# DarylFernandes99/custom-yolo-implmentation

Hardware: AMD Instinct MI355X
Metric: images/sec (640x640 bf16) (higher is better)
Workload: dtype bf16; 1 GPU; preset s (width 32..512, depth 1) 640x640 train step (fwd+DFL/QFL loss+bwd+grad sync+AdamW), COCO-80 synthetic, 32 img/GPU; global_batch=32, parallelism=dp1, hip_graph=True, optimizer_in_graph=True, deterministic_mode=False

## Files before the change

custom-yolo-implmentation_amd/csrc/elementwise.hip:

```cpp
#include "common.h"

namespace {

constexpr int TPB = 256;
constexpr int RS_ROWS = 2;
constexpr int RS_MAXBLK = 256 * 8;

template <typename T> __host__ bool vec_ok(const void* p, long ld, int C) {
    constexpr int V = vec_of<T>::N;
    return (C % V == 0) && (ld % V == 0) && ((reinterpret_cast<uintptr_t>(p) % 16) == 0);
}

template <typename TI, typename TO>
__global__ void k_ncm_to_nhwc(const TI* __restrict__ src, long sn, long sc, long off,
                              TO* __restrict__ dst, int ld, int C, int HW) {
    __shared__ float tile[32][33];
    const int n = blockIdx.z, p0 = blockIdx.x * 32, c0 = blockIdx.y * 32;
    const int tx = threadIdx.x & 31, ty = threadIdx.x >> 5;
    for (int r = ty; r < 32; r += 8) {
        int c = c0 + r, p = p0 + tx;
        tile[r][tx] = (c < C && p < HW) ? to_f<TI>(src[n * sn + c * sc + off + p]) : 0.f;
    }
    __syncthreads();
    for (int r = ty; r < 32; r += 8) {
        int p = p0 + r, c = c0 + tx;
        if (p < HW && c < C) dst[((long)n * HW + p) * ld + c] = from_f<TO>(tile[tx][r]);
    }
}

template <typename TI, typename TO>
__global__ void k_nhwc_to_ncm(const TI* __restrict__ src, int ld, TO* __restrict__ dst, long sn,
                              long sc, long off, int C, int HW) {
    __shared__ float tile[32][33];
// ... 121 lines not shown
        int cg = (int)(i - p * cv);
        float a[V];
        load_pack<T, V>(src + p * lds_ + cg * V, a);
        if (ACC) {
            float b[V];
            load_pack<T, V>(dst + p * ldd + cg * V, b);
#pragma unroll
            for (int j = 0; j < V; ++j) a[j] += b[j];
        }
        store_pack<T, V>(dst + p * ldd + cg * V, a);
    }
}

struct AddSrcs { const void* p[4]; int ld[4]; };
template <typename T, int V, int NS>
__global__ void k_add_n(AddSrcs s, T* __restrict__ dst, int ldd, long npix, int cv) {
    long total = npix * cv;
    for (long i = blockIdx.x * (long)blockDim.x + threadIdx.x; i < total; i += (long)gridDim.x * blockDim.x) {
        long p = i / cv;
        int cg = (int)(i - p * cv);
        float a[V];
        load_pack<T, V>((const T*)s.p[0] + p * s.ld[0] + cg * V, a);
#pragma unroll
        for (int k = 1; k < NS; ++k) {
            float b[V];
            load_pack<T, V>((const T*)s.p[k] + p * s.ld[k] + cg * V, b);
#pragma unroll
            for (int j = 0; j < V; ++j) a[j] += b[j];
        }
        store_pack<T, V>(dst + p * ldd + cg * V, a);
    }
}

__device__ __forceinline__ float sigmoid_rcp(float x) { return __builtin_amdgcn_rcpf(1.0f + __expf(-x)); }

__device__ __forceinline__ float act_grad(float z, int act) {
    if (act == 0) return 1.f;
    float s = sigmoid_rcp(z);
    return s * (1.f + z * (1.f - s));
}
__device__ __forceinline__ float act_fwd(float z, int act) { return act == 0 ? z : z * sigmoid_rcp(z); }

struct RsThread { int rpb, r, cl, cg; bool active; };
__device__ __forceinline__ RsThread rs_thread(int tpr, int cv) {
    RsThread t;
    t.rpb = TPB / tpr;
    t.r = threadIdx.x / tpr;
    t.cl = threadIdx.x - t.r * tpr;
    t.cg = blockIdx.y * tpr + t.cl;
    t.active = (t.r < t.rpb) && (t.cg < cv);
    return t;
}

template <typename T, int V, typename F>
__device__ __forceinline__ void rs_walk(const RsThread& t, const T* __restrict__ a, int lda, const T* __restrict__ b, int ldb, bool has_b,
                                        long npix, F one) {
    const long step = (long)gridDim.x * t.rpb;
    long p = (long)blockIdx.x * t.rpb + t.r;
    for (; p + (RS_ROWS - 1) * step < npix; p += RS_ROWS * step) {
        pack_t<T, V> ra[RS_ROWS], rb[RS_ROWS];
#pragma unroll
        for (int k = 0; k < RS_ROWS; ++k) {
            ra[k] = load_raw<T, V>(a + (p + k * step) * lda + t.cg * V);
            if (has_b) rb[k] = load_raw<T, V>(b + (p + k * step) * ldb + t.cg * V);
        }
#pragma unroll
        for (int k = 0; k < RS_ROWS; ++k) one(p + k * step, ra[k], rb[k]);
    }
#pragma clang loop vectorize(disable)
    for (; p < npix; p += step) {
        pack_t<T, V> pa = load_raw<T, V>(a + p * lda + t.cg * V), pb;
        if (has_b) pb = load_raw<T, V>(b + p * ldb + t.cg * V);
        one(p, pa, pb);
// ... 21 lines not shown
            unpack<T, V>(pa, a);
            if (MODE == 1) unpack<T, V>(pd, d);
#pragma unroll
            for (int j = 0; j < V; ++j) {
                if (MODE == 0) { s[j] += a[j]; q[j] += a[j] * a[j]; }
                else {
                    float dz = d[j] * act_grad(a[j] * sc[j] + sh[j], ACT);
                    s[j] += dz;
                    q[j] += dz * a[j];
                }
            }
        });
    }
#pragma unroll
    for (int j = 0; j < V; ++j) { red[threadIdx.x][j] = s[j]; red[threadIdx.x][V + j] = q[j]; }
    __syncthreads();
    for (int t = threadIdx.x; t < tpr * 2 * V; t += TPB) {
        const int cl = t / (2 * V), j = t - cl * 2 * V;
        float a = 0.f;
#pragma unroll 8
        for (int rr = 0; rr < th.rpb; ++rr) a += red[rr * tpr + cl][j];
        const int cgo = blockIdx.y * tpr + cl;
        if (cgo < cv) sink((j / V) * C + cgo * V + (j % V), a);
    }
}

template <typename T, int V, int MODE, int ACT>
__global__ __launch_bounds__(TPB) __attribute__((amdgpu_waves_per_eu(5, 8)))
void k_channel_reduce(const T* __restrict__ y, int ldy, const T* __restrict__ dout, int ldd, const float* __restrict__ scale,
                      const float* __restrict__ shift, long npix, int C, float* __restrict__ partial, int tpr) {
    float* o = partial + (long)blockIdx.x * 2 * C;
    channel_sums<T, V, MODE, ACT>(y, ldy, dout, ldd, scale, shift, npix, C, tpr, [&](int i, float a) { o[i] = a; });
}

struct PIn {
    const void* p; int dt;
    __device__ __forceinline__ float ld(int i) const {
        return dt == YOLO_F32 ? ((const float*)p)[i] : dt == YOLO_BF16 ? (float)((const bf16_t*)p)[i] : (float)((const f16_t*)p)[i];
    }
};
struct PIo {
    void* p; int dt;
    __device__ __forceinline__ float ld(int i) const {
        return dt == YOLO_F32 ? ((const float*)p)[i] : dt == YOLO_BF16 ? (float)((const bf16_t*)p)[i] : (float)((const f16_t*)p)[i];
    }
    __device__ __forceinline__ void st(int i, float v) const {
        if (dt == YOLO_F32) ((float*)p)[i] = v; else if (dt == YOLO_BF16) ((bf16_t*)p)[i] = (bf16_t)v; else ((f16_t*)p)[i] = (f16_t)v;
    }
};
static inline bool pdt_ok(int dt) { return dt == YOLO_F32 || dt == YOLO_BF16 || dt == YOLO_F16; }

constexpr int BN_REPL = 8;

extern __shared__ float cf[];

__device__ __forceinline__ void acc_fold(const float* __restrict__ acc, int C, int c, double& s, double& q) {
    s = 0.0; q = 0.0;
#pragma unroll
    for (int r = 0; r < BN_REPL; ++r) { s += acc[(long)r * 2 * C + c]; q += acc[(long)r * 2 * C + C + c]; }
}

template <typename T, int V, int MODE, int ACT>
__global__ __launch_bounds__(TPB) __attribute__((amdgpu_waves_per_eu(5, 8)))
void k_channel_acc(const T* __restrict__ y, int ldy, const T* __restrict__ dout, int ldd, const float* __restrict__ scale,
                   const float* __restrict__ shift, long npix, int C, float* __restrict__ acc, int tpr) {
    float* o = acc + (long)(blockIdx.x % BN_REPL) * 2 * C;
    channel_sums<T, V, MODE, ACT>(y, ldy, dout, ldd, scale, shift, npix, C, tpr, [&](int i, float a) { atomicAdd(o + i, a); });
}

struct BnFwdCoef { float mean, invstd, scale, shift, unbiased; };
__device__ __forceinline__ BnFwdCoef bn_fwd_coef(double s, double q, float count, float eps, float gamma, float beta) {
    const double m = s / count;
    double var = q / count - m * m;
    if (var < 0.0) var = 0.0;
    BnFwdCoef k;
    k.invstd = (float)(1.0 / sqrt(var + (double)eps));
    k.mean = (float)m;
    k.scale = gamma * k.invstd;
    k.shift = beta - (float)m * k.scale;
    k.unbiased = (float)(count > 1.f ? var * (count / (count - 1.0)) : var);
    return k;
}
__device__ __forceinline__ void bn_fwd_publish(const BnFwdCoef& k, int c, float momentum, float* __restrict__ mean,
                                               float* __restrict__ invstd, float* __restrict__ scale,
                                               float* __restrict__ shift, const PIo& rmean, const PIo& rvar) {
    mean[c] = k.mean;
    invstd[c] = k.invstd;
    scale[c] = k.scale;
    shift[c] = k.shift;
    if (rmean.p) {
        rmean.st(c, (1.f - momentum) * rmean.ld(c) + momentum * k.mean);
        rvar.st(c, (1.f - momentum) * rvar.ld(c) + momentum * k.unbiased);
    }
}
struct BnBwdCoef { float dbeta, dgamma, A, B, D; };
__device__ __forceinline__ BnBwdCoef bn_bwd_coef(double s, double q, float count, const PIn& gamma, const float* __restrict__ mean,
                                                 const float* __restrict__ invstd, int c) {
    const double is = invstd[c], mu = mean[c];
    q = is * (q - mu * s);
    const double k0 = (double)gamma.ld(c) * is, c1 = s / count, c2 = q / count;
    BnBwdCoef k;
    k.dbeta = (float)s;
    k.dgamma = (float)q;
    k.A = (float)k0;
    k.B = (float)(-k0 * c2 * is);
    k.D = (float)(-k0 * c1 + k0 * c2 * mu * is);
    return k;
}

__global__ void k_bn_finalize_acc(const float* __restrict__ acc, float count, int C, const void* __restrict__ gamma_,
                                  const void* __restrict__ beta_, void* __restrict__ rmean_, void* __restrict__ rvar_,
                                  float momentum, float eps, float* __restrict__ mean, float* __restrict__ invstd,
                                  float* __restrict__ scale, float* __restrict__ shift, int pdt, int bdt) {
    const PIn gamma{gamma_, pdt}; const PIn beta{beta_, pdt}; const PIo rmean{rmean_, bdt}, rvar{rvar_, bdt};
    const int c = blockIdx.x * blockDim.x + threadIdx.x;
    if (c >= C) return;
    double s, q;
    acc_fold(acc, C, c, s, q);
    bn_fwd_publish(bn_fwd_coef(s, q, count, eps, gamma.ld(c), beta.ld(c)), c, momentum, mean, invstd, scale, shift, rmean, rvar);
}

template <typename T, int V>
__device__ __forceinline__ void bn_act_fwd_rows(const RsThread& th, const T* __restrict__ y, int ldy, const T* __restrict__ res,
                                                int ldr, T* __restrict__ out, int ldo, long npix, const float (&sc)[V],
                                                const float (&sh)[V], int act) {
    const bool has_res = res;
    rs_walk<T, V>(th, y, ldy, res, ldr, has_res, npix, [&](long p, const pack_t<T, V>& pa, const pack_t<T, V>& pt) {
        float a[V], t[V];
        unpack<T, V>(pa, a);
        if (has_res) unpack<T, V>(pt, t);
#pragma unroll
        for (int j = 0; j < V; ++j) a[j] = act_fwd(a[j] * sc[j] + sh[j], act) + (has_res ? t[j] : 0.f);
        store_pack<T, V>(out + p * ldo + th.cg * V, a);
    });
}

template <typename T, int V>
__device__ __forceinline__ void bn_act_bwd_rows(const RsThread& th, const T* __restrict__ dout, int ldd, const T* __restrict__ y,
                                                int ldy, T* __restrict__ dy, int lddy, long npix, int cw, int act) {
    const float* my = cf + th.cl * V;
// ... 699 lines not shown
```

custom-yolo-implmentation_amd/csrc/stem.hip:

```cpp
#include "common.h"
#include "conv_dev.h"

namespace {

template <typename TI, typename TO>
__global__ void k_stem_im2col(const TI* __restrict__ img, TO* __restrict__ col, int N, int H, int W, int OH, int OW) {
    long total = (long)N * OH * OW;
    for (long p = blockIdx.x * (long)blockDim.x + threadIdx.x; p < total; p += (long)gridDim.x * blockDim.x) {
        int ow = (int)(p % OW);
        long t = p / OW;
        int oh = (int)(t % OH);
        long n = t / OH;
        float v[32];
#pragma unroll
        for (int k = 27; k < 32; ++k) v[k] = 0.f;
#pragma unroll
        for (int ci = 0; ci < 3; ++ci) {
            const TI* plane = img + (n * 3 + ci) * (long)H * W;
#pragma unroll
            for (int kh = 0; kh < 3; ++kh) {
                int ih = 2 * oh + kh - 1;
#pragma unroll
                for (int kw = 0; kw < 3; ++kw) {
                    int iw = 2 * ow + kw - 1;
                    bool ok = ih >= 0 && ih < H && iw >= 0 && iw < W;
                    v[ci * 9 + kh * 3 + kw] = ok ? to_f<TI>(plane[(long)ih * W + iw]) : 0.f;
                }
            }
        }
        TO* o = col + p * 32;
        constexpr int V = vec_of<TO>::N;
#pragma unroll
        for (int k = 0; k < 32; k += V) {
// ... 269 lines not shown
    const int e = blockIdx.x * 8 + (threadIdx.x >> 5), l = threadIdx.x & 31;
    if (e >= Cout * 27) return;
    const int o = e / 27, k = e - o * 27;
    float s = 0.f;
    for (int b = l; b < nslab; b += 32) s += part[((long)b * Cout + o) * 32 + k];
#pragma unroll
    for (int off = 16; off > 0; off >>= 1) s += __shfl_xor(s, off, 32);
    if (l == 0) dw[e] = from_f<P>(s);
}

constexpr int STEM_WG_SLABS = 1024;

template <typename T>
int launch_stem_wgrad(const float* img, const void* dy, int ldy, float* part, int N, int H, int W, int OH, int OW, int Cout,
                      int* nslab, hipStream_t st) {
    const long tiles = (long)N * ((OH + 1) / 2) * ((OW + STEM_SEG - 1) / STEM_SEG);
    if (tiles <= 0) return YOLO_ERR_ARG;
    const int grid = (int)(tiles < STEM_WG_SLABS ? tiles : STEM_WG_SLABS);
    *nslab = grid;
#define STEM_WG(CT) hipLaunchKernelGGL((k_stem_wgrad<T, CT>), dim3(grid), dim3(256), 0, st, img, (const T*)dy, ldy, part, N, H, W, OH, OW, tiles)
    switch (Cout / 16) {
        case 1: STEM_WG(1); break;
        case 2: STEM_WG(2); break;
        case 3: STEM_WG(3); break;
        case 4: STEM_WG(4); break;
        case 6: STEM_WG(6); break;
        case 8: STEM_WG(8); break;
        default: return YOLO_ERR_ARG;
    }
#undef STEM_WG
    return YOLO_LAUNCH_CHECK();
}

template <typename T>
int launch_stem_conv(const float* img, const void* wp, void* y, int ldy, float* stats, int N, int H, int W, int OH, int OW,
                     int Cout, const float* bias, int act, hipStream_t st) {
    const long blocks = (long)N * ((OH + 1) / 2) * ((OW + STEM_SEG - 1) / STEM_SEG);
    if (blocks <= 0 || blocks > 0x7fffffffL) return YOLO_ERR_ARG;
#define STEM_CT(CT) hipLaunchKernelGGL((k_stem_conv<T, CT>), dim3((unsigned)blocks), dim3(256), 0, st, img, (const T*)wp, (T*)y, ldy, stats, N, H, W, OH, OW, Cout, bias, act)
    switch (Cout / 16) {
        case 1: STEM_CT(1); break;
        case 2: STEM_CT(2); break;
        case 3: STEM_CT(3); break;
        case 4: STEM_CT(4); break;
        case 6: STEM_CT(6); break;
        case 8: STEM_CT(8); break;
        default: return YOLO_ERR_ARG;
    }
#undef STEM_CT
    return YOLO_LAUNCH_CHECK();
}

}

extern "C" {

int yolo_stem_im2col(const void* img, int img_dtype, void* col, int col_dtype, int N, int H, int W, int OH, int OW,
                     hipStream_t st) {
    if (OH != (H - 1) / 2 + 1 || OW != (W - 1) / 2 + 1) return YOLO_ERR_ARG;
    long total = (long)N * OH * OW;
    int grid = (int)((total + 255) / 256 > 256 * 16 ? 256 * 16 : (total + 255) / 256);
    if (grid < 1) grid = 1;
#define STEM_LAUNCH(TI) YOLO_DISPATCH_T(col_dtype, hipLaunchKernelGGL((k_stem_im2col<TI, T>), dim3(grid), dim3(256), 0, st, (const TI*)img, (T*)col, N, H, W, OH, OW))
    switch (img_dtype) {
        case YOLO_F32:  STEM_LAUNCH(float); break;
        case YOLO_BF16: STEM_LAUNCH(bf16_t); break;
// ... 34 lines not shown
           (ct == 1 || ct == 2 || ct == 3 || ct == 4 || ct == 6 || ct == 8);
}

int yolo_stem_conv_fwd(const float* img, const void* wp, void* y, int ldy, float* stats, int N, int H, int W, int OH, int OW,
                       int Cout, const float* bias, int act, int dtype, hipStream_t st) {
    if ((bias != nullptr || act) && stats != nullptr) return YOLO_ERR_ARG;
    if (act != 0 && act != 1) return YOLO_ERR_ARG;
    if (!yolo_stem_conv_eligible(YOLO_F32, dtype, Cout) || ldy < Cout) return YOLO_ERR_ARG;
    if (OH != (H - 1) / 2 + 1 || OW != (W - 1) / 2 + 1) return YOLO_ERR_ARG;
    if (dtype == YOLO_BF16) return launch_stem_conv<bf16_t>(img, wp, y, ldy, stats, N, H, W, OH, OW, Cout, bias, act, st);
    return launch_stem_conv<f16_t>(img, wp, y, ldy, stats, N, H, W, OH, OW, Cout, bias, act, st);
}

int yolo_stem_wgrad_slabs(void) { return STEM_WG_SLABS; }

int yolo_stem_wgrad(const float* img, const void* dy, int ldy, float* partial, void* dw, int dw_dtype, int N, int H, int W,
                    int OH, int OW, int Cout, int dtype, hipStream_t st) {
    if (!yolo_stem_conv_eligible(YOLO_F32, dtype, Cout) || ldy < Cout || (ldy & 7) || (reinterpret_cast<uintptr_t>(dy) & 15)) return YOLO_ERR_ARG;
    if (OH != (H - 1) / 2 + 1 || OW != (W - 1) / 2 + 1) return YOLO_ERR_ARG;
    int nslab = 0;
    const int rc = dtype == YOLO_BF16 ? launch_stem_wgrad<bf16_t>(img, dy, ldy, partial, N, H, W, OH, OW, Cout, &nslab, st)
                                      : launch_stem_wgrad<f16_t>(img, dy, ldy, partial, N, H, W, OH, OW, Cout, &nslab, st);
    if (rc) return rc;
    const int grid = (Cout * 27 + 7) / 8;
    switch (dw_dtype) {
        case YOLO_F32:  hipLaunchKernelGGL((k_stem_wgrad_reduce<float>), dim3(grid), dim3(256), 0, st, partial, nslab, Cout, (float*)dw); break;
        case YOLO_BF16: hipLaunchKernelGGL((k_stem_wgrad_reduce<bf16_t>), dim3(grid), dim3(256), 0, st, partial, nslab, Cout, (bf16_t*)dw); break;
        case YOLO_F16:  hipLaunchKernelGGL((k_stem_wgrad_reduce<f16_t>), dim3(grid), dim3(256), 0, st, partial, nslab, Cout, (f16_t*)dw); break;
        default: return YOLO_ERR_DTYPE;
    }
    return YOLO_LAUNCH_CHECK();
}

}
```

custom-yolo-implmentation_amd/src/hipops/functions.py:

```python
import contextlib
import os

import torch

from . import ops
from .lib import ACT_IDENTITY, ACT_SILU

_LOWP = (torch.bfloat16, torch.float16)


def compute_dtype(x, w):
    dev = x.device.type
    if torch.is_autocast_enabled(dev):
        return torch.get_autocast_dtype(dev)
    if w.dtype in _LOWP:
        return w.dtype
    return x.dtype if x.dtype in (torch.float32,) + _LOWP else torch.float32


def _as_nhwc(t, dtype):
    return t if (t.dtype == dtype and ops.is_nhwc(t)) else ops.to_nhwc(t, dtype)


def _f32(t):
# ... 251 lines not shown


def fanout(x, k):
    if k < 2 or not (torch.is_grad_enabled() and x.requires_grad):
        return (x,) * k
    return Fanout.apply(x, k)


def _on_fwd_stream(forward):
    def on_stream(ctx, *args):
        if FWD_STREAM is not None:
            with torch.cuda.stream(FWD_STREAM):
                return forward(ctx, *args)
        return forward(ctx, *args)
    return staticmethod(on_stream)


def _bn_act_grads(dout, y, saved, act, training, acc_b):
    scale, shift, mean, invstd, gamma = saved
    if training and acc_b is not None:
        return ops.bn_act_bwd_train(dout, y, scale, shift, mean, invstd, gamma, act, acc_b)
    if training:
        return ops.bn_act_bwd(dout, y, scale, shift, mean, invstd, gamma, act)
    return ops.bn_act_bwd_eval(dout, y, scale, shift, act), None, None


def _stem_grads(x, weight, dy, fused):
    def run(out=None):
        if fused:
            return ops.stem_wgrad(x, dy, weight.dtype, out)
        return ops.stem_unpack_wgrad(ops.conv_wgrad(x, dy, 1, 1, torch.float32), weight.dtype, out)
    lazy = x.is_cuda and LAZY_WGRAD_JOIN
    return _param_grad(x.device, weight.shape, weight.dtype, (x, dy), run) if lazy else run()


def _dw_grads(x, weight, dy, xshape, link, want_dx, want_dw):
    dx = dw = None
    if want_dx:
        dx = _fan_bwd(link, xshape, dy.dtype, lambda into: ops.dw_dgrad(dy, _f32(weight).reshape(-1, 9), acc_into=into))
    if want_dw:
        if weight.dtype == torch.float32 and x.is_cuda and LAZY_WGRAD_JOIN:
            dw = _param_grad(x.device, (x.shape[1], 1, 3, 3), torch.float32, (x, dy), lambda out: ops.dw_wgrad(x, dy, out=out))
        else:
            dw = ops.dw_wgrad(x, dy).to(weight.dtype)
    return dx, dw


def _dense_dgrad(weight, dy, xshape, k, stride, link):
    (n, cin, h, w), T = xshape, dy.dtype
    def run(acc_into, acc2=None):
        return ops.conv_dgrad(dy, ops.pack_weights(weight, k, stride, 1, T), cin, h, w, k, stride, acc_into=acc_into, acc2=acc2)
    if link is not None and link.chunk is not None and link.chunk.absorb(link, xshape, T, stride, run):
        return None
    return _fan_bwd(link, xshape, T, run, leaves=link is not None and link.fan)


def _dense_grads(x, weight, dy, xshape, k, stride, link, want_dx, want_dw):
    if want_dx and want_dw:
        return _wgrad_overlapped(x, dy, k, stride, weight.dtype, lambda: _dense_dgrad(weight, dy, xshape, k, stride, link))
    if want_dx:
        return _dense_dgrad(weight, dy, xshape, k, stride, link), None
    return None, (ops.conv_wgrad(x, dy, k, stride, weight.dtype) if want_dw else None)


class ConvBnAct(torch.autograd.Function):

# ... 22 lines not shown
            y = ops.dw_fwd(x, _f32(weight).reshape(cout, 9), acc_f)
        else:
            x = _as_nhwc(x, T)
            y = ops.conv_fwd(x, ops.pack_weights(weight, k, stride, 0, T), None, cout, k, stride, acc_f)
        rm, rv = bufs
        if res is not None:
            res = _as_nhwc(res, T)
        acc_b = None
        if training:
            if BnArena.current is not None and not deterministic:
                acc_b = BnArena.current.take(cout)
            if deterministic:
                mean, invstd, scale, shift = ops.bn_train_stats(y, gamma, beta, rm, rv, momentum, eps)
                out = ops.bn_act_fwd(y, scale, shift, act, res, out)
            else:
                out, mean, invstd, scale, shift = ops.bn_act_fwd_train(y, acc_f, gamma, beta, rm, rv, momentum, eps, act, res, out)
        else:
            mean = invstd = None
            scale, shift = ops.bn_eval_coeffs(gamma, beta, rm, rv, eps)
            out = ops.bn_act_fwd(y, scale, shift, act, res, out)
        saved = (scale, shift, mean, invstd, gamma)
        ctx.acc_b = acc_b
        ctx.cfg = (k, stride, depthwise, act, training, tuple(x.shape), res is not None, gamma.dtype, stem)
        ctx.stem_fused = stem_fused
        ctx.save_for_backward(x, weight, y, *saved)
        return _fresh(out)

    @staticmethod
    def backward(ctx, dout):
        k, stride, depthwise, act, training, xshape, has_res, gdtype, stem = ctx.cfg
        x, weight, y = ctx.saved_tensors[:3]
        T = y.dtype
        dout = _as_nhwc(dout, T)
        dy, dgamma, dbeta = _bn_act_grads(dout, y, ctx.saved_tensors[3:], act, training, ctx.acc_b)
        want_dx, want_dw = ctx.needs_input_grad[:2]
        link = ctx.res_link if not has_res else None
        if stem:
            dx, dw = None, (_stem_grads(x, weight, dy, ctx.stem_fused) if want_dw else None)
        elif depthwise:
            dx, dw = _dw_grads(x, weight, dy, xshape, link if (link is not None and link.fan) else None, want_dx, want_dw)
        else:
            dx, dw = _dense_grads(x, weight, dy, xshape, k, stride, link, want_dx, want_dw)
        if dgamma is None or not ctx.needs_input_grad[2]:
            dgamma = dbeta = None
        dres = dout if (has_res and ctx.needs_input_grad[4]) else None
        if has_res and ctx.res_link is not None and not ctx.res_link.fan:
            ctx.res_link.leave(dres)
        return dx, dw, dgamma, dbeta, dres, None, None, None, None, None, None, None, None, None, None


class ConvBias(torch.autograd.Function):

    @_on_fwd_stream
    def forward(ctx, x, weight, bias, k, stride):
        T = compute_dtype(x, weight)
        x = _as_nhwc(x, T)
        cout = weight.shape[0]
        b32 = _f32(bias) if bias is not None else None
        y = ops.conv_fwd(x, ops.pack_weights(weight, k, stride, 0, T), b32, cout, k, stride)
        ctx.cfg = (k, stride, tuple(x.shape), None if bias is None else bias.dtype)
        ctx.save_for_backward(x, weight)
        return y

    @staticmethod
    def backward(ctx, dy):
        k, stride, xshape, bdtype = ctx.cfg
        x, weight = ctx.saved_tensors
        dy = _as_nhwc(dy, x.dtype)
        n, cin, h, w = xshape
        dx = dw = db = None
# ... 298 lines not shown
```

custom-yolo-implmentation_amd/src/hipops/ops.py:

```python
import os

import torch

from . import lib

ALGO = int(os.environ.get("YOLO_HIP_CONV_ALGO", "0"))

_DT = {torch.float32: lib.F32, torch.bfloat16: lib.BF16, torch.float16: lib.F16}


def dt(t):
    try:
        return _DT[t.dtype if isinstance(t, torch.Tensor) else t]
    except KeyError:
        raise RuntimeError(f"unsupported dtype {t}")


def _stream(t):
    if not t.is_cuda:
        raise RuntimeError("yolo_hip ops need tensors on the GPU: the product path has no CPU fallback "
                           "(the CPU oracle lives under oracle/ and is test infrastructure)")
    return _raw_stream(t.device.index)


# ... 285 lines not shown
    oh, ow = (h - 1) // 2 + 1, (w - 1) // 2 + 1
    col = new_nhwc(n, 32, oh, ow, dtype, img.device) if out is None else out
    assert tuple(col.shape) == (n, 32, oh, ow) and col.dtype == dtype and geom(col)[4] == 32
    lib.call("yolo_stem_im2col", _p(img), dt(img), _p(col), dt(dtype), n, h, w, oh, ow, _stream(img))
    return col


def stem_conv_eligible(img, dtype, cout):
    return img.dtype == torch.float32 and dtype in _DT and \
        bool(lib.query("yolo_stem_conv_eligible", dt(img), dt(dtype), cout))


def stem_conv_fwd(img, wp, cout, dtype, stats_acc=None, bias=None, act=0):
    img = img if img.is_contiguous() else img.contiguous()
    n, c, h, w = img.shape
    assert c == 3
    oh, ow = (h - 1) // 2 + 1, (w - 1) // 2 + 1
    y = new_nhwc(n, cout, oh, ow, dtype, img.device)
    lib.call("yolo_stem_conv_fwd", _p(img), _p(wp), _p(y), cout, _p(stats_acc), n, h, w, oh, ow, cout, _p(bias), act, dt(dtype),
             _stream(img))
    return y


def stem_wgrad(img, dy, w_dtype, out=None):
    n, _, h, w = img.shape
    _, cout, oh, ow, ldy = geom(dy)
    dw = torch.empty((cout, 3, 3, 3), dtype=w_dtype, device=img.device) if out is None else out
    assert dw.shape == (cout, 3, 3, 3) and dw.dtype == w_dtype and dw.is_contiguous() and img.is_contiguous()
    part = torch.empty(lib.query("yolo_stem_wgrad_slabs") * cout * 32, dtype=torch.float32, device=img.device)
    lib.call("yolo_stem_wgrad", _p(img), _p(dy), ldy, _p(part), _p(dw), dt(w_dtype), n, h, w, oh, ow, cout, dt(dy), _stream(img))
    return dw


def stem_pack_weights(w, dtype):
    w = w if w.is_contiguous() else w.contiguous()
    out = torch.empty(w.shape[0] * 32, dtype=dtype, device=w.device)
    lib.call("yolo_stem_pack_weights", _p(w), dt(w), w.shape[0], _p(out), dt(dtype), _stream(w))
    return out


def stem_unpack_wgrad(dw32, w_dtype, out=None):
    cout = dw32.shape[0]
    dw = torch.empty((cout, 3, 3, 3), dtype=w_dtype, device=dw32.device) if out is None else out
    assert dw.shape == (cout, 3, 3, 3) and dw.dtype == w_dtype and dw.is_contiguous()
    lib.call("yolo_stem_unpack_wgrad", _p(dw32), cout, _p(dw), dt(w_dtype), _stream(dw32))
    return dw


def dw_fwd(x, w9, stats_acc=None):
    n, c, h, w, ldx = geom(x)
    y = new_nhwc(n, c, h, w, x.dtype, x.device)
    if stats_acc is not None:
        rc = lib.query("yolo_dwconv3x3_fwd_stats", _p(x), ldx, _p(w9), _p(y), c, _p(stats_acc), n, h, w, c, dt(x), _stream(x))
        if rc == 0:
            return y
        if rc != 1:
            lib.status(rc, "yolo_dwconv3x3_fwd_stats")
    lib.call("yolo_dwconv3x3_fwd", _p(x), ldx, _p(w9), _p(y), c, n, h, w, c, dt(x), _stream(x))
    if stats_acc is not None:
        bn_stats_acc(y, stats_acc)
    return y


def dw_fwd_act(x, w9, bias, act):
    n, c, h, w, ldx = geom(x)
    y = new_nhwc(n, c, h, w, x.dtype, x.device)
# ... 408 lines not shown
```

include/yolo_hip.h:

```cpp
#ifndef YOLO_HIP_H
#define YOLO_HIP_H
#include <stddef.h>
#include <stdint.h>

#ifdef __cplusplus
extern "C" {
#endif

#ifndef __HIP__
typedef struct ihipStream_t* hipStream_t;
#endif

#define YOLO_F32 0
#define YOLO_BF16 1
#define YOLO_F16 2
#define YOLO_ERR_ARG 1001
#define YOLO_ERR_DTYPE 1002
#define YOLO_ACT_IDENTITY 0
#define YOLO_ACT_SILU 1

long yolo_abi_hash(void);

int yolo_memset0(void* p, size_t bytes, hipStream_t st);
int yolo_ncm_to_nhwc(const void* src, int src_dtype, long sn, long sc, long off, void* dst, int dst_dtype, int ld, int N, int C, int HW, hipStream_t st);
// ... 19 lines not shown
int yolo_adamw_step(const void* jobs_dev, int njobs, long nchunks, const double* hyper, float* step, const float* grad_scale, const float* found_inf, hipStream_t st);
int yolo_adamw_job_set_ema(void* jobs_host, int index, float* ema, double* ema_ctl);
int yolo_ema_lerp(const void* jobs_dev, int njobs, long nchunks, const double* ema_ctl, const float* skip_flag, hipStream_t st);
int yolo_adamw_amp_step(const void* jobs_dev, int njobs, long nchunks, const double* hyper, float* step, float* amp_state, int* growth_tracker, float growth_factor, float backoff_factor, int growth_interval, hipStream_t st);
int yolo_grad_sqnorm(const void* jobs_dev, int njobs, long nchunks, float* partials, float* found_inf, hipStream_t st);
int yolo_grad_clip_finalize(const float* partials, long nparts, float* clip_state, const float* grad_scale, hipStream_t st);
int yolo_adamw_clip_step(const void* jobs_dev, int njobs, long nchunks, const double* hyper, float* step, const float* grad_scale, const float* found_inf, const float* clip_state, hipStream_t st);
int yolo_amp_update_scale(float* amp_state, int* growth_tracker, float growth_factor, float backoff_factor, int growth_interval, hipStream_t st);
int yolo_sgd_step(const void* jobs_dev, int njobs, long nchunks, const double* hyper, float* step, const float* grad_scale, const float* found_inf, const float* clip_state, hipStream_t st);
int yolo_sgd_amp_step(const void* jobs_dev, int njobs, long nchunks, const double* hyper, float* step, float* amp_state, int* growth_tracker, float growth_factor, float backoff_factor, int growth_interval, hipStream_t st);
int yolo_copy_job_bytes();
int yolo_copy_job_fill(void* jobs_host, int index, const void* src, int src_dtype, void* dst, int dst_dtype, long n);
long yolo_copy_jobs_finalize(void* jobs_host, int njobs);
int yolo_multi_copy(const void* jobs_dev, int njobs, long nchunks, float scale, hipStream_t st);
int yolo_conv2d_fwd(const void* x, int ldx, const void* wp, const float* bias, void* y, int ldy, float* stats_acc, int N, int H, int W, int Cin, int OH, int OW, int Cout, int k, int stride, int dtype, int algo, hipStream_t st);
int yolo_conv2d_fwd_act(const void* x, int ldx, const void* wp, const float* bias, const void* res, int ldr, void* y, int ldy, int N, int H, int W, int Cin, int OH, int OW, int Cout, int k, int stride, int act, int dtype, hipStream_t st);
int yolo_conv2d_dgrad(const void* dy, int lddy, const void* wb, void* dx, int lddx, int N, int H, int W, int Cin, int OH, int OW, int Cout, int k, int stride, int accumulate, int dtype, int algo, hipStream_t st);
int yolo_conv2d_dgrad_acc2(const void* dy, int lddy, const void* wb, void* dx, int lddx, const void* acc2, int ld2, int N, int H, int W, int Cin, int OH, int OW, int Cout, int k, int stride, int dtype, int algo, hipStream_t st);
long yolo_conv2d_wgrad_ws_elems(const void* x, int ldx, const void* dy, int ldy, int N, int H, int W, int Cin, int OH, int OW, int Cout, int k, int stride, int dtype, int algo);
int yolo_conv2d_wgrad(const void* x, int ldx, const void* dy, int ldy, float* ws, void* dw_oihw, int dw_dtype, int N, int H, int W, int Cin, int OH, int OW, int Cout, int k, int stride, int dtype, int algo, hipStream_t st);
int yolo_conv_tune_set(int bn, int tap_inner, int halo, int dma, int ring, int bm, int nst, int bk);
int yolo_wgrad_tune_set(int to, int ti, int blocks, int min_per);
int yolo_wgrad_tune_pf(int pf);
int yolo_conv_wide_set(int on);
int yolo_conv2d_plan(int N, int H, int W, int Cin, int OH, int OW, int Cout, int k, int stride, int mode, int cls, int dtype);
long yolo_conv2d_wgrad_plan(int N, int H, int W, int Cin, int OH, int OW, int Cout, int k, int stride, int dtype);
int yolo_stem_im2col(const void* img, int img_dtype, void* col, int col_dtype, int N, int H, int W, int OH, int OW, hipStream_t st);
int yolo_stem_pack_weights(const void* w, int w_dtype, int Cout, void* out, int out_dtype, hipStream_t st);
int yolo_stem_unpack_wgrad(const float* dw32, int Cout, void* dw, int dw_dtype, hipStream_t st);
int yolo_stem_conv_eligible(int img_dtype, int dtype, int Cout);
int yolo_stem_conv_fwd(const float* img, const void* wp, void* y, int ldy, float* stats, int N, int H, int W, int OH, int OW, int Cout, const float* bias, int act, int dtype, hipStream_t st);
int yolo_stem_wgrad_slabs();
int yolo_stem_wgrad(const float* img, const void* dy, int ldy, float* partial, void* dw, int dw_dtype, int N, int H, int W, int OH, int OW, int Cout, int dtype, hipStream_t st);
int yolo_dwconv3x3_fwd(const void* x, int ldx, const float* w, void* y, int ldy, int N, int H, int W, int C, int dtype, hipStream_t st);
int yolo_dwconv3x3_fwd_stats(const void* x, int ldx, const float* w, void* y, int ldy, float* stats, int N, int H, int W, int C, int dtype, hipStream_t st);
int yolo_dwconv3x3_fwd_act(const void* x, int ldx, const float* w, const float* bias, void* y, int ldy, int N, int H, int W, int C, int act, int dtype, hipStream_t st);
int yolo_dwconv3x3_dgrad(const void* dy, int lddy, const float* w, void* dx, int lddx, int N, int H, int W, int C, int accumulate, int dtype, hipStream_t st);
int yolo_dw_wgrad_nslab(int N, int H);
int yolo_dwconv3x3_wgrad(const void* x, int ldx, const void* dy, int ldy, float* dw, float* partial, int N, int H, int W, int C, int dtype, hipStream_t st);
int yolo_dw_tune_set(int variant);
int yolo_dw_plan(int N, int H, int W, int C, int field);

int yolo_reduce_nblk(long npix, int C);
int yolo_bn_stats(const void* y, int ldy, long npix, int C, int dtype, float* partial, int nblk, hipStream_t st);
int yolo_bn_finalize(const float* partial, int nblk, long count, int C, const void* gamma, const void* beta, void* running_mean, void* running_var, float momentum, float eps, float* mean, float* invstd, float* scale, float* shift, int pdtype, int bdtype, hipStream_t st);
int yolo_bn_eval_coeffs(const void* gamma, const void* beta, const void* running_mean, const void* running_var, float eps, int C, float* scale, float* shift, int pdtype, int bdtype, hipStream_t st);
int yolo_sum_finalize(const float* partial, int nblk, int C, float* out, hipStream_t st);
int yolo_bn_act_fwd(const void* y, int ldy, const float* scale, const float* shift, const void* res, int ldres, void* out, int ldout, long npix, int C, int act, int dtype, hipStream_t st);
int yolo_bn_act_bwd_reduce(const void* dout, int ldd, const void* y, int ldy, const float* scale, const float* shift, const float* mean, const float* invstd, long npix, int C, int act, int dtype, float* partial, int nblk, hipStream_t st);
int yolo_bn_bwd_finalize(const float* partial, int nblk, long count, int C, const void* gamma, const float* mean, const float* invstd, void* dgamma, void* dbeta, float* coef, int pdtype, hipStream_t st);
int yolo_bn_act_bwd_apply(const void* dout, int ldd, const void* y, int ldy, const float* scale, const float* shift, const float* mean, const float* invstd, const float* coef, void* dy, int lddy, long npix, int C, int act, int dtype, hipStream_t st);
int yolo_bn_acc_elems(int C);
int yolo_bn_stats_acc(const void* y, int ldy, long npix, int C, int dtype, float* acc, hipStream_t st);
int yolo_bn_finalize_acc(const float* acc, long count, int C, const void* gamma, const void* beta, void* running_mean, void* running_var, float momentum, float eps, float* mean, float* invstd, float* scale, float* shift, int pdtype, int bdtype, hipStream_t st);
int yolo_bn_act_fwd_train(const void* y, int ldy, const float* acc, long count, const void* gamma, const void* beta, void* running_mean, void* running_var, float momentum, float eps, float* mean, float* invstd, float* scale, float* shift, const void* res, int ldres, void* out, int ldout, long npix, int C, int act, int dtype, int pdtype, int bdtype, hipStream_t st);
int yolo_bn_bwd_reduce_acc(const void* dout, int ldd, const void* y, int ldy, const float* scale, const float* shift, long npix, int C, int act, int dtype, float* acc, hipStream_t st);
int yolo_bn_act_bwd_apply_train(const void* dout, int ldd, const void* y, int ldy, const float* scale, const float* shift, const void* gamma, const float* mean, const float* invstd, const float* acc, long count, void* dgamma, void* dbeta, void* dy, int lddy, long npix, int C, int act, int dtype, int pdtype, hipStream_t st);

int yolo_maxpool5_fwd(const void* x, int ldx, void* out, int ldo, uint8_t* idx, int N, int H, int W, int C, int dtype, hipStream_t st);
int yolo_maxpool5_bwd(const void* dout, int ldd, const uint8_t* idx, void* dx, int ldx, int N, int H, int W, int C, int accumulate, int dtype, hipStream_t st);
int yolo_upsample2x_fwd(const void* x, int ldx, void* out, int ldo, int N, int H, int W, int C, int dtype, hipStream_t st);
int yolo_upsample2x_bwd(const void* dout, int ldd, void* dx, int ldx, int N, int H, int W, int C, int accumulate, int dtype, hipStream_t st);

size_t yolo_attn_stash_bytes(int N, int T_, int heads, int dtype);
size_t yolo_attn_workspace_bytes(int N, int T_, int heads, int dtype);
size_t yolo_attn_stash_bytes_for(int N, int T, int heads, int dk, int dh, int dtype);
// ... 48 lines not shown
```

Measured before the change: 3073 images/s.

## Fuse stem BN-activation backward with weight-gradient into one pass

Adds a stem backward kernel that reads dout and y once, computes the BN/activation pre-gradient on the fly, and accumulates two MFMA products (dz·x and y·x) plus per-channel sums. A finalize kernel then folds in the BN backward coefficients algebraically to produce dw, dgamma and dbeta. This removes the separate BN backward reduce/apply passes and the materialized dy tensor for the stem layer, which works at the largest spatial resolution. In exchange it does more MFMA work and carries a larger partial-sum workspace with a double-precision finalize.

```diff
diff --git a/custom-yolo-implmentation_amd/csrc/bn_coef.h b/custom-yolo-implmentation_amd/csrc/bn_coef.h
--- /dev/null
+++ b/custom-yolo-implmentation_amd/csrc/bn_coef.h
@@ -0,0 +1,54 @@
+#pragma once
+#include "common.h"
+
+__device__ __forceinline__ float sigmoid_rcp(float x) { return __builtin_amdgcn_rcpf(1.0f + __expf(-x)); }
+
+__device__ __forceinline__ float act_grad(float z, int act) {
+    if (act == 0) return 1.f;
+    float s = sigmoid_rcp(z);
+    return s * (1.f + z * (1.f - s));
+}
+
+struct PIn {
+    const void* p; int dt;
+    __device__ __forceinline__ float ld(int i) const {
+        return dt == YOLO_F32 ? ((const float*)p)[i] : dt == YOLO_BF16 ? (float)((const bf16_t*)p)[i] : (float)((const f16_t*)p)[i];
+    }
+};
+struct PIo {
+    void* p; int dt;
+    __device__ __forceinline__ float ld(int i) const {
+        return dt == YOLO_F32 ? ((const float*)p)[i] : dt == YOLO_BF16 ? (float)((const bf16_t*)p)[i] : (float)((const f16_t*)p)[i];
+    }
+    __device__ __forceinline__ void st(int i, float v) const {
+        if (dt == YOLO_F32) ((float*)p)[i] = v; else if (dt == YOLO_BF16) ((bf16_t*)p)[i] = (bf16_t)v; else ((f16_t*)p)[i] = (f16_t)v;
+    }
+};
+static inline bool pdt_ok(int dt) { return dt == YOLO_F32 || dt == YOLO_BF16 || dt == YOLO_F16; }
+
+struct BnBwdCoefD { double dbeta, dgamma, A, B, D; };
+__device__ __forceinline__ BnBwdCoefD bn_bwd_coef_d(double s, double q, float count, const PIn& gamma, const float* __restrict__ mean,
+                                                    const float* __restrict__ invstd, int c) {
+    const double is = invstd[c], mu = mean[c];
+    q = is * (q - mu * s);
+    const double k0 = (double)gamma.ld(c) * is, c1 = s / count, c2 = q / count;
+    BnBwdCoefD k;
+    k.dbeta = s;
+    k.dgamma = q;
+    k.A = k0;
+    k.B = -k0 * c2 * is;
+    k.D = -k0 * c1 + k0 * c2 * mu * is;
+    return k;
+}
+struct BnBwdCoef { float dbeta, dgamma, A, B, D; };
+__device__ __forceinline__ BnBwdCoef bn_bwd_coef(double s, double q, float count, const PIn& gamma, const float* __restrict__ mean,
+                                                 const float* __restrict__ invstd, int c) {
+    const BnBwdCoefD d = bn_bwd_coef_d(s, q, count, gamma, mean, invstd, c);
+    BnBwdCoef k;
+    k.dbeta = (float)d.dbeta;
+    k.dgamma = (float)d.dgamma;
+    k.A = (float)d.A;
+    k.B = (float)d.B;
+    k.D = (float)d.D;
+    return k;
+}
diff --git a/custom-yolo-implmentation_amd/csrc/elementwise.hip b/custom-yolo-implmentation_amd/csrc/elementwise.hip
--- a/custom-yolo-implmentation_amd/csrc/elementwise.hip
+++ b/custom-yolo-implmentation_amd/csrc/elementwise.hip
@@ -1,4 +1,5 @@
 #include "common.h"
+#include "bn_coef.h"
 
 namespace {
 
@@ -186,13 +187,6 @@
     }
 }
 
-__device__ __forceinline__ float sigmoid_rcp(float x) { return __builtin_amdgcn_rcpf(1.0f + __expf(-x)); }
-
-__device__ __forceinline__ float act_grad(float z, int act) {
-    if (act == 0) return 1.f;
-    float s = sigmoid_rcp(z);
-    return s * (1.f + z * (1.f - s));
-}
 __device__ __forceinline__ float act_fwd(float z, int act) { return act == 0 ? z : z * sigmoid_rcp(z); }
 
 struct RsThread { int rpb, r, cl, cg; bool active; };
@@ -280,23 +274,6 @@
     float* o = partial + (long)blockIdx.x * 2 * C;
     channel_sums<T, V, MODE, ACT>(y, ldy, dout, ldd, scale, shift, npix, C, tpr, [&](int i, float a) { o[i] = a; });
 }
-
-struct PIn {
-    const void* p; int dt;
-    __device__ __forceinline__ float ld(int i) const {
-        return dt == YOLO_F32 ? ((const float*)p)[i] : dt == YOLO_BF16 ? (float)((const bf16_t*)p)[i] : (float)((const f16_t*)p)[i];
-    }
-};
-struct PIo {
-    void* p; int dt;
-    __device__ __forceinline__ float ld(int i) const {
-        return dt == YOLO_F32 ? ((const float*)p)[i] : dt == YOLO_BF16 ? (float)((const bf16_t*)p)[i] : (float)((const f16_t*)p)[i];
-    }
-    __device__ __forceinline__ void st(int i, float v) const {
-        if (dt == YOLO_F32) ((float*)p)[i] = v; else if (dt == YOLO_BF16) ((bf16_t*)p)[i] = (bf16_t)v; else ((f16_t*)p)[i] = (f16_t)v;
-    }
-};
-static inline bool pdt_ok(int dt) { return dt == YOLO_F32 || dt == YOLO_BF16 || dt == YOLO_F16; }
 
 constexpr int BN_REPL = 8;
 
@@ -340,20 +317,6 @@
         rmean.st(c, (1.f - momentum) * rmean.ld(c) + momentum * k.mean);
         rvar.st(c, (1.f - momentum) * rvar.ld(c) + momentum * k.unbiased);
     }
-}
-struct BnBwdCoef { float dbeta, dgamma, A, B, D; };
-__device__ __forceinline__ BnBwdCoef bn_bwd_coef(double s, double q, float count, const PIn& gamma, const float* __restrict__ mean,
-                                                 const float* __restrict__ invstd, int c) {
-    const double is = invstd[c], mu = mean[c];
-    q = is * (q - mu * s);
-    const double k0 = (double)gamma.ld(c) * is, c1 = s / count, c2 = q / count;
-    BnBwdCoef k;
-    k.dbeta = (float)s;
-    k.dgamma = (float)q;
-    k.A = (float)k0;
-    k.B = (float)(-k0 * c2 * is);
-    k.D = (float)(-k0 * c1 + k0 * c2 * mu * is);
-    return k;
 }
 
 __global__ void k_bn_finalize_acc(const float* __restrict__ acc, float count, int C, const void* __restrict__ gamma_,
diff --git a/custom-yolo-implmentation_amd/csrc/stem.hip b/custom-yolo-implmentation_amd/csrc/stem.hip
--- a/custom-yolo-implmentation_amd/csrc/stem.hip
+++ b/custom-yolo-implmentation_amd/csrc/stem.hip
@@ -1,4 +1,5 @@
 #include "common.h"
+#include "bn_coef.h"
 #include "conv_dev.h"
 
 namespace {
@@ -334,6 +335,252 @@
     return YOLO_LAUNCH_CHECK();
 }
 
+constexpr int STEM_BN_SLABS = 512;
+constexpr long stem_bn_block(int cout) { return (long)cout * 64 + 32 + 2 * cout; }
+
+template <typename T, int CT, int ACT>
+__global__ __launch_bounds__(256) void k_stem_bn_wgrad(const float* __restrict__ img, const T* __restrict__ dout, int ldd,
+                                                       const T* __restrict__ y, int ldy, const float* __restrict__ scale,
+                                                       const float* __restrict__ shift, float* __restrict__ part, int N, int H,
+                                                       int W, int OH, int OW, long tiles) {
+    typedef mfma_ops<T> ops;
+    typedef typename ops::frag frag;
+    typedef pack_t<T, 8> chunk;
+    constexpr int LDY = stem_ldy(CT), COUT = 16 * CT, TILE = 2 * STEM_SEG * LDY;
+    constexpr int CPP = COUT / 8, PPT = 256 / CPP, NP = (2 * STEM_SEG + PPT - 1) / PPT;
+    constexpr int RED = 17;
+    static_assert((2 * COUT * 32 + 32 + 256 * RED) * sizeof(float) <= 2 * TILE * sizeof(T), "the sums reuse the two tiles");
+    __shared__ __attribute__((aligned(16))) float rows[3 * STEM_IR][STEM_ROWW + 7];
+    __shared__ __attribute__((aligned(16))) T zs[2 * TILE];
+    const int tid = threadIdx.x, lane = tid & 63, wave = tid >> 6;
+    const int g = lane >> 4, i16 = lane & 15, q4 = i16 >> 2, c4 = 4 * (i16 & 3);
+    const int segs = (OW + STEM_SEG - 1) / STEM_SEG, ohp = (OH + 1) >> 1;
+    const int cpc = tid % CPP, pl = tid / CPP;
+    const bool mine = pl < PPT;
+    f32x4 acc1[CT][2], acc2[CT][2];
+#pragma unroll
+    for (int ct = 0; ct < CT; ++ct)
+#pragma unroll
+        for (int nt = 0; nt < 2; ++nt) acc1[ct][nt] = acc2[ct][nt] = (f32x4){0.f, 0.f, 0.f, 0.f};
+    float g3[2] = {0.f, 0.f}, s[8], q[8], sc[8], sh[8];
+#pragma unroll
+    for (int j = 0; j < 8; ++j) {
+        s[j] = q[j] = 0.f;
+        sc[j] = scale[cpc * 8 + j];
+        sh[j] = shift[cpc * 8 + j];
+    }
+    int krow[2], kcol[2];
+#pragma unroll
+    for (int nt = 0; nt < 2; ++nt) {
+        const int k = nt * 16 + i16, ci = k / 9, r3 = k / 3;
+        krow[nt] = k < 27 ? ci * STEM_IR + (r3 - ci * 3) : -1;
+        kcol[nt] = k - r3 * 3 + 3;
+    }
+    chunk dv[NP], yv[NP];
+    auto fetch = [&](long tl) {
+        const int seg = (int)(tl % segs);
+        const long t = tl / segs;
+        const int oh0 = (int)(t % ohp) * 2, n = (int)(t / ohp), ow0 = seg * STEM_SEG;
+#pragma unroll
+        for (int k = 0; k < NP; ++k) {
+            const int px = pl + k * PPT, j = px / STEM_SEG, p = px - j * STEM_SEG;
+            const bool ok = mine && px < 2 * STEM_SEG && oh0 + j < OH && ow0 + p < OW;
+            const long pix = ((long)n * OH + (ok ? oh0 + j : 0)) * OW + (ok ? ow0 + p : 0);
+            dv[k] = load_raw<T, 8>(dout + pix * ldd + cpc * 8);
+            yv[k] = load_raw<T, 8>(y + pix * ldy + cpc * 8);
+            if (!ok) dv[k] = yv[k] = chunk{};
+        }
+    };
+    if (blockIdx.x < tiles) fetch(blockIdx.x);
+    for (long tl = blockIdx.x; tl < tiles; tl += gridDim.x) {
+        const int seg = (int)(tl % segs);
+        const long t = tl / segs;
+        const int oh0 = (int)(t % ohp) * 2, n = (int)(t / ohp);
+        const int ow0 = seg * STEM_SEG, iw0 = 2 * ow0 - 1;
+        __syncthreads();
+        constexpr int RPW = (3 * STEM_IR + 3) / 4;
+        float4 v[RPW];
+        float edge[RPW];
+        const bool w4 = (W & 3) == 0;
+        if (w4) {
+            const int c = lane * 4;
+#pragma unroll
+            for (int k = 0; k < RPW; ++k) {
+                const int r = wave + 4 * k, rr = r < 3 * STEM_IR ? r : 0;
+                const int ci = rr / STEM_IR, ir = rr - ci * STEM_IR;
+                const int ih = 2 * oh0 + ir - 1;
+                const bool rok = ih >= 0 && ih < H;
+                const float* src = img + (((long)n * 3 + ci) * H + (rok ? ih : 0)) * (long)W + 2 * ow0;
+                const bool cok = 2 * ow0 + c < W;
+                v[k] = *reinterpret_cast<const float4*>(src + (cok ? c : 0));
+                if (!(rok && cok)) v[k] = make_float4(0.f, 0.f, 0.f, 0.f);
+                edge[k] = (lane == 0 && ow0 > 0) ? src[-1] : 0.f;
+                if (!rok) edge[k] = 0.f;
+            }
+        }
+#pragma unroll
+        for (int k = 0; k < NP; ++k) {
+            const int px = pl + k * PPT;
+            if (mine && px < 2 * STEM_SEG) {
+                float d[8], a[8];
+                unpack<T, 8>(dv[k], d);
+                unpack<T, 8>(yv[k], a);
+                chunk z;
+#pragma unroll
+                for (int j = 0; j < 8; ++j) {
+                    const float dz = d[j] * act_grad(a[j] * sc[j] + sh[j], ACT);
+                    s[j] += dz;
+                    q[j] += dz * a[j];
+                    z.v[j] = from_f<T>(dz);
+                }
+                *reinterpret_cast<chunk*>(zs + px * LDY + cpc * 8) = z;
+                *reinterpret_cast<chunk*>(zs + TILE + px * LDY + cpc * 8) = yv[k];
+            }
+        }
+        if (w4) {
+            const int c = lane * 4;
+#pragma unroll
+            for (int k = 0; k < RPW; ++k) {
+                const int r = wave + 4 * k;
+                if (r < 3 * STEM_IR) {
+                    *reinterpret_cast<float4*>(&rows[r][4 + c]) = v[k];
+                    if (lane == 0) rows[r][3] = edge[k];
+                }
+            }
+        } else {
+            for (int idx = tid; idx < 3 * STEM_IR * STEM_ROWW; idx += 256) {
+                const int r = idx / STEM_ROWW, c = idx - r * STEM_ROWW;
+                const int ci = r / STEM_IR, ir = r - ci * STEM_IR;
+                const int ih = 2 * oh0 + ir - 1, iw = iw0 + c;
+                const bool ok = ih >= 0 && ih < H && iw >= 0 && iw < W;
+                rows[r][3 + c] = ok ? img[(((long)n * 3 + ci) * H + ih) * (long)W + iw] : 0.f;
+            }
+        }
+        if (tl + gridDim.x < tiles) fetch(tl + gridDim.x);
+        __syncthreads();
+#pragma unroll
+        for (int j = 0; j < 2; ++j) {
+            const int px0 = wave * 32;
+            const bool rowok = oh0 + j < OH;
+            frag fb[2];
+#pragma unroll
+            for (int nt = 0; nt < 2; ++nt) {
+#pragma unroll
+                for (int e = 0; e < 8; ++e) {
+                    const float x = krow[nt] >= 0 ? rows[krow[nt] < 0 ? 0 : krow[nt] + 2 * j][2 * (px0 + 8 * g + e) + kcol[nt]] : 0.f;
+                    const T xr = from_f<T>(x);
+                    fb[nt][e] = xr;
+                    g3[nt] += (rowok && ow0 + px0 + 8 * g + e < OW) ? to_f<T>(xr) : 0.f;
+                }
+            }
+#pragma unroll
+            for (int ct = 0; ct < CT; ++ct) {
+                const T* p = zs + (j * STEM_SEG + px0 + 8 * g + q4) * LDY + ct * 16 + c4;
+                const frag fz = stem_tr_frag<T>(p, p + 4 * LDY);
+                const frag fy = stem_tr_frag<T>(p + TILE, p + TILE + 4 * LDY);
+#pragma unroll
+                for (int nt = 0; nt < 2; ++nt) {
+                    acc1[ct][nt] = ops::mma(fz, fb[nt], acc1[ct][nt]);
+                    acc2[ct][nt] = ops::mma(fy, fb[nt], acc2[ct][nt]);
+                }
+            }
+        }
+    }
+    float* sum = reinterpret_cast<float*>(zs);
+    float* g3s = sum + 2 * COUT * 32;
+    float* red = g3s + 32;
+#pragma unroll
+    for (int nt = 0; nt < 2; ++nt) {
+        g3[nt] += __shfl_xor(g3[nt], 16, 64);
+        g3[nt] += __shfl_xor(g3[nt], 32, 64);
+    }
+    for (int wv = 0; wv < 4; ++wv) {
+        __syncthreads();
+        if (wave == wv) {
+#pragma unroll
+            for (int ct = 0; ct < CT; ++ct)
+#pragma unroll
+                for (int nt = 0; nt < 2; ++nt)
+#pragma unroll
+                    for (int r = 0; r < 4; ++r) {
+                        float* e = &sum[(ct * 16 + g * 4 + r) * 32 + nt * 16 + i16];
+                        e[0] = wv == 0 ? acc1[ct][nt][r] : e[0] + acc1[ct][nt][r];
+                        e[COUT * 32] = wv == 0 ? acc2[ct][nt][r] : e[COUT * 32] + acc2[ct][nt][r];
+                    }
+            if (g == 0) {
+#pragma unroll
+                for (int nt = 0; nt < 2; ++nt) g3s[nt * 16 + i16] = wv == 0 ? g3[nt] : g3s[nt * 16 + i16] + g3[nt];
+            }
+        }
+    }
+#pragma unroll
+    for (int j = 0; j < 8; ++j) { red[tid * RED + j] = s[j]; red[tid * RED + 8 + j] = q[j]; }
+    __syncthreads();
+    float* o = part + (long)blockIdx.x * stem_bn_block(COUT);
+    for (int c = tid; c < 2 * COUT * 32 + 32; c += 256) o[c] = sum[c];
+    for (int t = tid; t < 2 * COUT; t += 256) {
+        const int which = t / COUT, ch = t - which * COUT, cl = ch >> 3, j = ch & 7;
+        float a = 0.f;
+        for (int rr = 0; rr < PPT; ++rr) a += red[(rr * CPP + cl) * RED + which * 8 + j];
+        o[2 * COUT * 32 + 32 + t] = a;
+    }
+}
+
+template <typename P>
+__global__ __launch_bounds__(1024) void k_stem_bn_wgrad_finalize(const float* __restrict__ part, int nslab, int Cout, float count,
+                                                                 const void* __restrict__ gamma_, const float* __restrict__ mean,
+                                                                 const float* __restrict__ invstd, void* __restrict__ dgamma_,
+                                                                 void* __restrict__ dbeta_, P* __restrict__ dw, int pdt) {
+    __shared__ double red[5][32][33];
+    const PIn gamma{gamma_, pdt}; const PIo dgamma{dgamma_, pdt}, dbeta{dbeta_, pdt};
+    const int co = blockIdx.x, k = threadIdx.x & 31, sub = threadIdx.x >> 5;
+    const long bs = stem_bn_block(Cout);
+    double a[5] = {0.0, 0.0, 0.0, 0.0, 0.0};
+#pragma unroll 4
+    for (int b = sub; b < nslab; b += 32) {
+        const float* p = part + b * bs;
+        a[0] += p[co * 32 + k];
+        a[1] += p[(Cout + co) * 32 + k];
+        a[2] += p[Cout * 64 + k];
+        a[3] += p[Cout * 64 + 32 + co];
+        a[4] += p[Cout * 64 + 32 + Cout + co];
+    }
+#pragma unroll
+    for (int i = 0; i < 5; ++i) red[i][sub][k] = a[i];
+    __syncthreads();
+    if (sub != 0) return;
+#pragma unroll
+    for (int i = 0; i < 5; ++i) {
+        double t = 0.0;
+        for (int j = 0; j < 32; ++j) t += red[i][j][k];
+        a[i] = t;
+    }
+    const BnBwdCoefD c = bn_bwd_coef_d(a[3], a[4], count, gamma, mean, invstd, co);
+    if (k == 0) { dbeta.st(co, (float)c.dbeta); dgamma.st(co, (float)c.dgamma); }
+    if (k < 27) dw[co * 27 + k] = from_f<P>((float)(c.A * a[0] + c.B * a[1] + c.D * a[2]));
+}
+
+template <typename T, int ACT>
+int launch_stem_bn_wgrad(const float* img, const void* dout, int ldd, const void* y, int ldy, const float* scale,
+                         const float* shift, float* part, int N, int H, int W, int OH, int OW, int Cout, int* nslab, hipStream_t st) {
+    const long tiles = (long)N * ((OH + 1) / 2) * ((OW + STEM_SEG - 1) / STEM_SEG);
+    if (tiles <= 0) return YOLO_ERR_ARG;
+    const int grid = (int)(tiles < STEM_BN_SLABS ? tiles : STEM_BN_SLABS);
+    *nslab = grid;
+#define STEM_BW(CT) hipLaunchKernelGGL((k_stem_bn_wgrad<T, CT, ACT>), dim3(grid), dim3(256), 0, st, img, (const T*)dout, ldd, (const T*)y, ldy, scale, shift, part, N, H, W, OH, OW, tiles)
+    switch (Cout / 16) {
+        case 1: STEM_BW(1); break;
+        case 2: STEM_BW(2); break;
+        case 3: STEM_BW(3); break;
+        case 4: STEM_BW(4); break;
+        case 6: STEM_BW(6); break;
+        case 8: STEM_BW(8); break;
+        default: return YOLO_ERR_ARG;
+    }
+#undef STEM_BW
+    return YOLO_LAUNCH_CHECK();
+}
+
 template <typename T>
 int launch_stem_conv(const float* img, const void* wp, void* y, int ldy, float* stats, int N, int H, int W, int OH, int OW,
                      int Cout, const float* bias, int act, hipStream_t st) {
@@ -434,4 +681,32 @@
     return YOLO_LAUNCH_CHECK();
 }
 
-}
+long yolo_stem_bn_wgrad_ws_elems(int Cout) { return STEM_BN_SLABS * stem_bn_block(Cout); }
+
+int yolo_stem_bn_wgrad(const float* img, const void* dout, int ldd, const void* y, int ldy, const float* scale, const float* shift,
+                       const void* gamma, const float* mean, const float* invstd, float* partial, void* dw, int dw_dtype,
+                       void* dgamma, void* dbeta, int N, int H, int W, int OH, int OW, int Cout, int act, int dtype, int pdt,
+                       hipStream_t st) {
+    if (!yolo_stem_conv_eligible(YOLO_F32, dtype, Cout) || !pdt_ok(pdt) || (act != 0 && act != 1)) return YOLO_ERR_ARG;
+    if (ldd < Cout || (ldd & 7) || (reinterpret_cast<uintptr_t>(dout) & 15)) return YOLO_ERR_ARG;
+    if (ldy < Cout || (ldy & 7) || (reinterpret_cast<uintptr_t>(y) & 15)) return YOLO_ERR_ARG;
+    if (OH != (H - 1) / 2 + 1 || OW != (W - 1) / 2 + 1) return YOLO_ERR_ARG;
+    int nslab = 0, rc;
+#define STEM_BW_ACT(T) (act ? launch_stem_bn_wgrad<T, 1>(img, dout, ldd, y, ldy, scale, shift, partial, N, H, W, OH, OW, Cout, &nslab, st) \
+                            : launch_stem_bn_wgrad<T, 0>(img, dout, ldd, y, ldy, scale, shift, partial, N, H, W, OH, OW, Cout, &nslab, st))
+    rc = dtype == YOLO_BF16 ? STEM_BW_ACT(bf16_t) : STEM_BW_ACT(f16_t);
+#undef STEM_BW_ACT
+    if (rc) return rc;
+    const float count = (float)((long)N * OH * OW);
+#define STEM_BW_FIN(P) hipLaunchKernelGGL((k_stem_bn_wgrad_finalize<P>), dim3(Cout), dim3(1024), 0, st, partial, nslab, Cout, count, gamma, mean, invstd, dgamma, dbeta, (P*)dw, pdt)
+    switch (dw_dtype) {
+        case YOLO_F32:  STEM_BW_FIN(float); break;
+        case YOLO_BF16: STEM_BW_FIN(bf16_t); break;
+        case YOLO_F16:  STEM_BW_FIN(f16_t); break;
+        default: return YOLO_ERR_DTYPE;
+    }
+#undef STEM_BW_FIN
+    return YOLO_LAUNCH_CHECK();
+}
+
+}
diff --git a/custom-yolo-implmentation_amd/src/hipops/functions.py b/custom-yolo-implmentation_amd/src/hipops/functions.py
--- a/custom-yolo-implmentation_amd/src/hipops/functions.py
+++ b/custom-yolo-implmentation_amd/src/hipops/functions.py
@@ -307,6 +307,14 @@
         return ops.stem_unpack_wgrad(ops.conv_wgrad(x, dy, 1, 1, torch.float32), weight.dtype, out)
     lazy = x.is_cuda and LAZY_WGRAD_JOIN
     return _param_grad(x.device, weight.shape, weight.dtype, (x, dy), run) if lazy else run()
+
+
+STEM_BWD_FUSED = os.environ.get("YOLO_STEM_BWD_FUSED", "1") == "1"
+
+
+def _stem_bn_grads(x, weight, dout, y, saved, act):
+    scale, shift, mean, invstd, gamma = saved
+    return ops.stem_bn_wgrad(x, dout, y, scale, shift, mean, invstd, gamma, act, weight.dtype)
 
 
 def _dw_grads(x, weight, dy, xshape, link, want_dx, want_dw):
@@ -395,10 +403,14 @@
         x, weight, y = ctx.saved_tensors[:3]
         T = y.dtype
         dout = _as_nhwc(dout, T)
-        dy, dgamma, dbeta = _bn_act_grads(dout, y, ctx.saved_tensors[3:], act, training, ctx.acc_b)
         want_dx, want_dw = ctx.needs_input_grad[:2]
         link = ctx.res_link if not has_res else None
-        if stem:
+        one_pass = stem and ctx.stem_fused and training and want_dw and STEM_BWD_FUSED
+        if not one_pass:
+            dy, dgamma, dbeta = _bn_act_grads(dout, y, ctx.saved_tensors[3:], act, training, ctx.acc_b)
+        if one_pass:
+            dx, (dw, dgamma, dbeta) = None, _stem_bn_grads(x, weight, dout, y, ctx.saved_tensors[3:], act)
+        elif stem:
             dx, dw = None, (_stem_grads(x, weight, dy, ctx.stem_fused) if want_dw else None)
         elif depthwise:
             dx, dw = _dw_grads(x, weight, dy, xshape, link if (link is not None and link.fan) else None, want_dx, want_dw)
diff --git a/custom-yolo-implmentation_amd/src/hipops/ops.py b/custom-yolo-implmentation_amd/src/hipops/ops.py
--- a/custom-yolo-implmentation_amd/src/hipops/ops.py
+++ b/custom-yolo-implmentation_amd/src/hipops/ops.py
@@ -341,6 +341,20 @@
     return dw
 
 
+def stem_bn_wgrad(img, dout, y, scale, shift, mean, invstd, gamma, act, w_dtype, out=None):
+    n, _, h, w = img.shape
+    _, cout, oh, ow, ldy = geom(y)
+    ldd = geom(dout)[4]
+    dw = torch.empty((cout, 3, 3, 3), dtype=w_dtype, device=img.device) if out is None else out
+    assert dw.shape == (cout, 3, 3, 3) and dw.dtype == w_dtype and dw.is_contiguous() and img.is_contiguous()
+    assert tuple(dout.shape) == tuple(y.shape) and dout.dtype == y.dtype
+    part = torch.empty(lib.query("yolo_stem_bn_wgrad_ws_elems", cout), dtype=torch.float32, device=img.device)
+    dgamma, dbeta = torch.empty_like(gamma), torch.empty_like(gamma)
+    lib.call("yolo_stem_bn_wgrad", _p(img), _p(dout), ldd, _p(y), ldy, _p(scale), _p(shift), _p(gamma), _p(mean), _p(invstd),
+             _p(part), _p(dw), dt(w_dtype), _p(dgamma), _p(dbeta), n, h, w, oh, ow, cout, int(act), dt(y), dt(gamma), _stream(img))
+    return dw, dgamma, dbeta
+
+
 def stem_pack_weights(w, dtype):
     w = w if w.is_contiguous() else w.contiguous()
     out = torch.empty(w.shape[0] * 32, dtype=dtype, device=w.device)
diff --git a/include/yolo_hip.h b/include/yolo_hip.h
--- a/include/yolo_hip.h
+++ b/include/yolo_hip.h
@@ -75,6 +75,8 @@
 int yolo_stem_conv_fwd(const float* img, const void* wp, void* y, int ldy, float* stats, int N, int H, int W, int OH, int OW, int Cout, const float* bias, int act, int dtype, hipStream_t st);
 int yolo_stem_wgrad_slabs();
 int yolo_stem_wgrad(const float* img, const void* dy, int ldy, float* partial, void* dw, int dw_dtype, int N, int H, int W, int OH, int OW, int Cout, int dtype, hipStream_t st);
+long yolo_stem_bn_wgrad_ws_elems(int Cout);
+int yolo_stem_bn_wgrad(const float* img, const void* dout, int ldd, const void* y, int ldy, const float* scale, const float* shift, const void* gamma, const float* mean, const float* invstd, float* partial, void* dw, int dw_dtype, void* dgamma, void* dbeta, int N, int H, int W, int OH, int OW, int Cout, int act, int dtype, int pdt, hipStream_t st);
 int yolo_dwconv3x3_fwd(const void* x, int ldx, const float* w, void* y, int ldy, int N, int H, int W, int C, int dtype, hipStream_t st);
 int yolo_dwconv3x3_fwd_stats(const void* x, int ldx, const float* w, void* y, int ldy, float* stats, int N, int H, int W, int C, int dtype, hipStream_t st);
 int yolo_dwconv3x3_fwd_act(const void* x, int ldx, const float* w, const float* bias, void* y, int ldy, int N, int H, int W, int C, int act, int dtype, hipStream_t st);
```

Result: faster. 3110 images/s (median of 6 runs) (+1.2%).
